# open-policy-agent/gatekeeper

Measured on AMD Instinct MI355X. Metric: AdmissionReview x constraint evals/sec, higher is better.
Workload: dtype u32; 1 GPU; configs[2]: pkg/audit sweep, 50 constraints x 1000000 mixed synthetic cluster objects (80% Pod, 10% Deployment, 5% Namespace, 5% Service/ConfigMap); constraints=50, reviews_total=1000000, reviews_rank0=1000000, rows_rank0=15859334, table_bytes_rank0=529437232, parallelism=1 GPU

## Files before the change

gatekeeper_amd/_lib.py:

```python
from __future__ import annotations

import atexit
import ctypes as C
import os

_HERE = os.path.dirname(os.path.abspath(__file__))
_ROOT = os.path.dirname(_HERE)

GK_OK = 0
GK_ERR_INVALID, GK_ERR_REGO, GK_ERR_UNSUPPORTED, GK_ERR_NOT_FOUND, GK_ERR_DEVICE, GK_ERR_REVIEW, GK_ERR_INTERNAL, GK_ERR_LIMIT = (
    -1, -2, -3, -4, -5, -6, -7, -8)
GK_REVIEW_ADMISSION_REQUEST, GK_REVIEW_OBJECT = 0, 1
GK_SRC_EMPTY, GK_SRC_ORIGINAL, GK_SRC_GENERATED, GK_SRC_ALL, GK_SRC_INVALID = 0, 1, 2, 3, 4
GK_TABLE_KEEP_DOCS = 1
GK_TABLE_RESIDENT = 2
GK_TABLE_KEEP_TEXT = 16
GK_TABLE_PRUNED = 32
GK_TABLE_PRE_MATCHED = 64
GK_TABLE_PROCESS_AUDIT = 4
GK_TABLE_PROCESS_WEBHOOK = 8
GK_REVIEW_EXCLUDED = 1
GK_EVAL_WANT_MATCH, GK_EVAL_NO_DOWNLOAD, GK_EVAL_WANT_LIST, GK_EVAL_ASYNC, GK_EVAL_COLLECT, GK_EVAL_TIME_EACH, GK_EVAL_KERNEL_ONLY = 1, 2, 4, 8, 16, 32, 64
GK_EVAL_DEVICE_ONLY = 128
GK_SWEEP_RESULT_TOTALS = 1

EXPORTS = [
    "gk_engine_create", "gk_engine_destroy", "gk_last_error", "gk_version", "gk_template_add", "gk_template_remove",
    "gk_constraint_add", "gk_constraint_remove", "gk_data_put", "gk_data_remove", "gk_excluder_replace", "gk_excluder_excluded", "gk_table_create", "gk_table_free",
    "gk_table_eval", "gk_eval_free", "gk_render", "gk_render_error", "gk_free", "gk_dump", "gk_table_topk", "gk_topk_free",
    "gk_table_totals", "gk_totals_free", "gk_table_get_stats", "gk_batcher_start", "gk_batcher_stop", "gk_query", "gk_query_ex", "gk_query_ex2",
    "gk_resident_sweep", "gk_sweep_free", "gk_resident_review", "gk_resident_review_ex",
    "gk_comm_unique_id", "gk_comm_init", "gk_comm_destroy", "gk_comm_info", "gk_table_sweep_sharded", "gk_shard_free",
    "gk_jit_quiesce", "gk_jit_cache_stats", "gk_jit_cache_dir", "gk_jit_cache_drop_memory", "gk_host_cpus", "gk_table_create_spool", "gk_spool_info_free", "gk_debug_set",
    "gk_synth_batch_create", "gk_synth_batch_reviews", "gk_synth_batch_size", "gk_synth_batch_json_bytes", "gk_synth_batch_free", "gk_synth_query_storm", "gk_synth_query_storm_ex",
]


GK_OPT_NO_REFERENTIAL, GK_OPT_GATHER_STATS, GK_OPT_TRACE = 1, 2, 4
GK_QUERY_TRACE = 1
GK_QUERY_PRE_MATCHED = 2


class gk_opts(C.Structure):
    _fields_ = [("device", C.c_int32), ("elem_cap", C.c_uint16 * 3), ("reserved", C.c_uint16), ("flags", C.c_uint32), ("reserved2", C.c_uint32),
                ("disabled_builtins", C.POINTER(C.c_char_p)), ("n_disabled_builtins", C.c_size_t)]


class gk_review_in(C.Structure):
    _fields_ = [("kind", C.c_int32), ("source", C.c_int32),
                ("json", C.c_char_p), ("json_len", C.c_size_t),
                ("namespace_json", C.c_char_p), ("namespace_len", C.c_size_t),
                ("ns_object_json", C.c_char_p), ("ns_object_len", C.c_size_t),
                ("operation", C.c_char_p)]


class gk_eval_out(C.Structure):
# ... 139 lines not shown
    lib.gk_topk_free.restype = None
    lib.gk_comm_unique_id.argtypes = [C.c_char_p]
    lib.gk_comm_init.argtypes = [vp, C.c_char_p, C.c_int, C.c_int]
    lib.gk_comm_destroy.argtypes = [vp]
    lib.gk_comm_destroy.restype = None
    lib.gk_comm_info.argtypes = [vp, C.POINTER(C.c_int32), C.POINTER(C.c_int32)]
    lib.gk_table_sweep_sharded.argtypes = [vp, vp, u32, C.POINTER(C.POINTER(gk_shard_out))]
    lib.gk_shard_free.argtypes = [C.POINTER(gk_shard_out)]
    lib.gk_shard_free.restype = None
    if hostemu:
        lib.gk_comm_init_host.argtypes = [vp, C.c_int, C.c_int, HE_ALLGATHER, HE_ALLREDUCE, vp]
    lib.gk_resident_sweep.argtypes = [vp, u32, C.POINTER(C.POINTER(gk_sweep_out))]
    lib.gk_sweep_free.argtypes = [C.POINTER(gk_sweep_out)]
    lib.gk_sweep_free.restype = None
    lib.gk_resident_review.argtypes = [vp, C.POINTER(cp), sz, C.POINTER(vp)]
    lib.gk_batcher_start.argtypes = [vp, C.POINTER(gk_batch_opts)]
    lib.gk_batcher_stop.argtypes = [vp]
    lib.gk_batcher_stop.restype = None
    lib.gk_query.argtypes = [vp, C.POINTER(gk_review_in), C.POINTER(vp), C.POINTER(gk_query_stats)]
    lib.gk_query_ex.argtypes = [vp, C.POINTER(gk_review_in), u32, C.POINTER(vp), C.POINTER(vp), C.POINTER(gk_query_stats)]
    lib.gk_query_ex2.argtypes = [vp, C.POINTER(gk_review_in), C.POINTER(u32), sz, u32, C.POINTER(vp), C.POINTER(vp), C.POINTER(gk_query_stats)]
    lib.gk_resident_review_ex.argtypes = [vp, C.POINTER(cp), sz, C.POINTER(u32), sz, u32, C.POINTER(vp)]
    lib.gk_debug_set.argtypes = [cp, C.c_int64]
    lib.gk_table_get_stats.argtypes = [vp, C.POINTER(gk_table_stats)]
    lib.gk_table_totals.argtypes = [vp, vp, C.POINTER(C.POINTER(gk_totals_out))]
    lib.gk_totals_free.argtypes = [C.POINTER(gk_totals_out)]
    lib.gk_totals_free.restype = None
    lib.gk_synth_batch_create.argtypes = [C.c_uint64, C.c_uint64, C.c_uint64, C.c_int, C.POINTER(cp), sz, C.POINTER(vp)]
    lib.gk_synth_batch_reviews.argtypes = [vp]
    lib.gk_synth_batch_reviews.restype = C.POINTER(gk_review_in)
    lib.gk_synth_batch_size.argtypes = [vp]
    lib.gk_synth_batch_size.restype = sz
    lib.gk_synth_batch_json_bytes.argtypes = [vp]
    lib.gk_synth_batch_json_bytes.restype = C.c_uint64
    lib.gk_synth_batch_free.argtypes = [vp]
    lib.gk_synth_batch_free.restype = None
    lib.gk_synth_query_storm.argtypes = [vp, vp, u32, u32, C.POINTER(gk_storm_out)]
    lib.gk_synth_query_storm_ex.argtypes = [vp, vp, u32, u32, C.POINTER(u32), sz, u32, C.POINTER(gk_storm_out)]
    atexit.register(lib.gk_jit_quiesce)
    _cache[hostemu] = lib
    return lib
```

gatekeeper_amd/csrc/device.hpp:

```cpp
#pragma once
#include <cstdint>
#include <string>
#include <vector>

#include "flatten.hpp"
#include "lower.hpp"

namespace gk {

struct DevTable;
struct DevPlan;

struct EvalOptions {
  bool download = true;
  bool want_match = false;
  uint32_t list_capacity = 0;
  bool shard = false;
  bool detached = false;
  bool kernel_only = false;
  bool time_each = false;
  bool timed = true;
  bool jit_wait = true;
};

// ... 39 lines not shown
int dev_comm_rank(const DevComm* c);
int dev_comm_world(const DevComm* c);
bool dev_comm_query(const DevComm* c, int* rank, int* world, std::string* err);
struct ShardInfo {
  uint32_t stride_tiles = 0;
  uint64_t slot_bytes = 0;
  std::vector<uint32_t> shard_reviews;
};
void dev_shard_setup(DevTable* t, DevComm* c, uint32_t nc, ShardInfo* info);
void dev_shard_exchange(DevTable* t, DevComm* c, uint32_t nc, uint64_t not_evaluated, std::vector<int64_t>* totals,
                        std::vector<uint64_t>* gathered , const void** d_gathered);
struct ShardExchangeStats { float exchange_ms = 0; uint64_t inbound_bytes = 0; bool overlap = false; };
ShardExchangeStats dev_shard_exchange_stats(const DevTable* t, const DevComm* c);
void dev_shard_enqueue(const DevPlan* p, DevTable* t, DevComm* c, const EvalOptions& opt, uint32_t nc, uint64_t not_evaluated, bool allow_graph);
bool dev_shard_collect(DevTable* t, DevComm* c, uint32_t nc, std::vector<int64_t>* totals, std::vector<uint64_t>* gathered, const void** d_gathered);
void dev_jit_quiesce();
void dev_jit_cache_stats(uint64_t* hits, uint64_t* compiles);
void dev_jit_cache_drop_memory();
const char* dev_jit_cache_dir();
void dev_jit_prefetch(const DevPlan* p, const DevTable* t);
void dev_eval_launch(const DevPlan* p, const DevTable* t, const EvalOptions& opt);
void dev_eval_finish(const DevPlan* p, const DevTable* t, const EvalOptions& opt, EvalOut* out);

}
```

gatekeeper_amd/csrc/engine.cpp:

```cpp
#include <atomic>
#include <cstring>
#include <dirent.h>
#include <algorithm>
#include <chrono>
#include <condition_variable>
#include <deque>
#include <functional>
#include <thread>
#include <map>
#include <unordered_map>
#include <unordered_set>
#include <memory>
#include <mutex>
#include <shared_mutex>
#include <sstream>

#include "../../include/gkgpu.h"
#include "codegen.hpp"
#include "device.hpp"
#include "flatten.hpp"
#include "lower.hpp"
#include "pe.hpp"
#include "regex.hpp"

// ... 232 lines not shown
    bool is_namespace = false, alive = true;
    uint32_t chunk = UINT32_MAX, slot = 0;
  };
  struct ResChunk {
    gk_table* table = nullptr;
    std::vector<uint32_t> obj_of_slot;
    std::vector<uint64_t> live;
    std::vector<uint64_t> shown;
    uint64_t excl_gen = 0;
    gk_eval_out* ev = nullptr;
    uint64_t plan_gen = 0;
    uint64_t n_live = 0;
  };
  struct Resident {
    std::mutex mu;
    std::vector<ResObj> objs;
    std::unordered_map<std::string, uint32_t> by_key;
    std::unordered_map<std::string, std::vector<uint32_t>> by_ns;
    std::unordered_map<uint64_t, uint32_t> by_text;
    std::vector<uint32_t> pending;
    std::vector<ResChunk> chunks;
    bool swept = false;
    uint64_t n_live = 0, n_dead_slots = 0, flattened_total = 0;
  } resident;
  struct BatchResult;
  struct Request {
    const gk_review_in* in = nullptr;
    bool pre_matched = false;
    std::chrono::steady_clock::time_point arrived;
    int status = GK_OK;
    std::string error;
    std::shared_ptr<BatchResult> batch;
    uint32_t index = 0;
    uint32_t batch_size = 0;
    double queue_us = 0, device_us = 0;
    bool done = false;
    std::condition_variable cv;
  };
  struct Batcher {
    std::mutex mu;
    std::condition_variable cv;
    std::deque<Request*> queue;
    std::vector<std::thread> workers;
    bool running = false, stop = false;
    gk_batch_opts opts{64, 200, 0, 0};
    uint64_t batches = 0, reviews = 0;
// ... 2006 lines not shown
        c.obj_of_slot.push_back(id);
      }
      R.pending.clear();
      if (!ins.empty()) {
        std::vector<int32_t> st(ins.size(), GK_OK);
        int rc = gk_table_create(e, ins.data(), ins.size(), GK_TABLE_RESIDENT | GK_TABLE_PRUNED, st.data(), &c.table);
        if (rc != GK_OK) return rc;
        c.live.assign((ins.size() + 63) / 64, 0);
        for (size_t k = 0; k < ins.size(); k++) {
          gk_engine::ResObj& o = R.objs[c.obj_of_slot[k]];
          o.chunk = (uint32_t)R.chunks.size(); o.slot = (uint32_t)k;
          if (st[k] == GK_OK) { c.live[k / 64] |= 1ull << (k % 64); c.n_live++; }
        }
        flattened = ins.size();
        R.flattened_total += flattened;
        R.chunks.push_back(std::move(c));
      }
    }
    const auto t1 = std::chrono::steady_clock::now();
    ensure_plan(e);
    uint64_t gen;
    { std::shared_lock<std::shared_mutex> l(e->plan_rw); gen = e->plan_gen; }
    std::unique_ptr<SweepHolder> h(new SweepHolder());
    for (auto& c : R.chunks) {
      if (c.ev && c.plan_gen == gen) continue;
      if (c.ev) { gk_eval_free(c.ev); c.ev = nullptr; }
      int rc = gk_table_eval(e, c.table, 0, &c.ev);
      if (rc != GK_OK) return rc;
      c.plan_gen = gen;
    }
    {
      std::shared_lock<std::shared_mutex> l(e->mu);
      auto ex = e->excluder.find("audit");
      for (auto& c : R.chunks) {
        if (c.excl_gen == e->excluder_gen && c.shown.size() == c.live.size()) {
          for (size_t w = 0; w < c.live.size(); w++) c.shown[w] &= c.live[w];
          continue;
        }
        c.shown = c.live;
        if (ex != e->excluder.end() && !ex->second.empty())
          for (size_t k = 0; k < c.obj_of_slot.size(); k++) {
            const gk_engine::ResObj& o = R.objs[c.obj_of_slot[k]];
            if (excluder_matches(ex->second, o.is_namespace ? o.path.back() : o.ns)) c.shown[k / 64] &= ~(1ull << (k % 64));
          }
        c.excl_gen = e->excluder_gen;
      }
    }
    if (!R.chunks.empty()) {
      const gk_eval_out* ev0 = R.chunks[0].ev;
      h->ids.assign(ev0->constraint_ids, ev0->constraint_ids + ev0->n_constraints);
    } else {
      { std::lock_guard<std::mutex> gate(e->plan_gate); }
// ... 293 lines not shown
    stats->total_us = std::chrono::duration<double, std::micro>(std::chrono::steady_clock::now() - req.arrived).count();
  }
  if (req.status != GK_OK) return fail(req.status, req.error);
  char* buf = (char*)malloc(results.size() + 1);
  memcpy(buf, results.c_str(), results.size() + 1);
  *results_json = buf;
  gk_query_stats mine{};
  mine.batch_size = req.batch_size; mine.queue_us = req.queue_us; mine.device_us = req.device_us;
  put_trace(on_host ? (pre_matched ? "by the host evaluator (the review is beyond the device's limits; pre-matched by the caller: violation sets by the concrete evaluator)"
                                   : "by the host evaluator (the review is beyond the device's limits: match layer from the stripped review on the device, violation sets by the concrete evaluator)")
                    : (pre_matched ? "on the device (pre-matched by the caller: violation bitmaps of the batch's one launch; messages rendered by the host evaluator for the flagged pairs)"
                                   : "on the device (match + violation bitmaps of the batch's one launch; messages rendered by the host evaluator for the flagged pairs)"), results, &mine);
  return GK_OK;
}

int gk_debug_set(const char* key, int64_t value) {
  if (!key) return fail(GK_ERR_INVALID, "NULL argument");
  if (strcmp(key, "dict_facts") == 0) { g_debug_dict_facts.store(value != 0); return GK_OK; }
  if (strcmp(key, "group_max") == 0) { g_debug_group_max.store((int)std::max<int64_t>(0, std::min<int64_t>(value, 1 << 20))); return GK_OK; }
  if (strcmp(key, "fold_match_labels") == 0) { g_test_fold_match_labels.store(value != 0); return GK_OK; }
  return fail(GK_ERR_NOT_FOUND, std::string("gk_debug_set: unknown key ") + key);
}

void gk_jit_quiesce(void) { dev_jit_quiesce(); }
void gk_jit_cache_drop_memory(void) { dev_jit_cache_drop_memory(); }
const char* gk_jit_cache_dir(void) { return dev_jit_cache_dir(); }
void gk_jit_cache_stats(uint64_t* cache_hits, uint64_t* compiles) {
  uint64_t h = 0, c = 0;
  dev_jit_cache_stats(&h, &c);
  if (cache_hits) *cache_hits = h;
  if (compiles) *compiles = c;
}

int gk_dump(gk_engine* e, char** text_out) {
  if (!e || !text_out) return fail(GK_ERR_INVALID, "NULL argument");
  try {
    ensure_plan(e);
    std::ostringstream os;
    std::shared_lock<std::shared_mutex> l(e->plan_rw);
    const HostPlan& p = e->fast;
    os << "constraints=" << p.dims.n_constraints << " viol_formulas=" << p.n_viol << " match_formulas=" << p.n_match
       << " preds=" << p.dims.n_preds << " scopes=" << p.dims.n_scopes << " code_words=" << p.dims.n_code
       << " gwords=" << p.dims.n_gwords << " acc_words=" << p.dims.acc_words << " lds_bytes_per_64_reviews=" << p.dims.acc_words * 256
       << " paths=" << p.dims.n_paths << "\n";
    for (size_t i = 0; i < p.preds.size(); i++)
      os << "pred " << i << " op=" << (int)p.preds[i].op << " dst=" << (int)p.preds[i].dst << " scope=" << (int)p.preds[i].scope
// ... 15 lines not shown
```

gatekeeper_amd/csrc/kernels.hip:

```cpp
#include <hip/hip_runtime.h>
#include <hip/hiprtc.h>
#include <dlfcn.h>
#include <sys/stat.h>
#include <sys/wait.h>
#include <spawn.h>
#include <unistd.h>
#include <fcntl.h>
#include <array>
#include <cstring>
#include <cerrno>
#include <set>

#include <cstdio>
#include <cstdlib>
#include <atomic>
#include <condition_variable>
#include <list>
#include <map>
#include <thread>
#include <memory>
#include <mutex>
#include <stdexcept>
#include <string>
#include <vector>

extern char** environ;

#include "chunks.hpp"
#include "codegen.hpp"
#include "device.hpp"
#include "jit_source.hpp"
#include "shard_pipe.hpp"
#include "jit_sources.inc"
#include "vm_core.hpp"

namespace gk {

#define HIP_OK(expr)                                                                                          \
  do {                                                                                                        \
    hipError_t e_ = (expr);                                                                                   \
    if (e_ != hipSuccess) throw std::runtime_error(std::string("HIP error: ") + hipGetErrorString(e_) + " at " #expr); \
  } while (0)

namespace {
struct DevPool {
  std::mutex mu;
  std::map<size_t, std::vector<void*>> free_;
  std::map<void*, size_t> class_of;
  size_t cached = 0;
};
DevPool& pool() { static DevPool p; return p; }
constexpr size_t kPoolMaxBlock = 32u << 20, kPoolMaxCached = 2048ull << 20;
std::mutex g_hip_alloc_mu;
hipError_t hip_malloc_serial(void** out, size_t bytes) { std::lock_guard<std::mutex> l(g_hip_alloc_mu); return hipMalloc(out, bytes); }
void hip_free_serial(void* p) { std::lock_guard<std::mutex> l(g_hip_alloc_mu); (void)hipFree(p); }
// ... 899 lines not shown
  void lc_release_more() {
    for (size_t k = 0; k < lc_more.size(); k++) { if (lc_pinned) pinned_release(reinterpret_cast<uint8_t*>(lc_more[k]), lc_more_cap[k]); else pool_free(lc_more[k]); }
    lc_more.clear(); lc_more_cap.clear(); lc_used = 0;
  }
  struct Launch {
    uint64_t plan = 0;
    bool want_match = false;
    hipFunction_t fn = nullptr;
    uint32_t grid = 0, block = 0, lds = 0, tot_k = 0;
    uint64_t kernel_hash = 0;
    PlanView pv{};
    const Row* rows = nullptr; const StrHdr* shdr = nullptr; const ChunkDesc* lists = nullptr; const uint32_t* rflags = nullptr; const uint8_t* heap = nullptr;
    const ConstraintSlot* slots = nullptr;
    uint32_t cg = 0, nn = 0, nt = 0, dd = 0, rp = 0;
    OutPtrs out{};
  } cached;
  bool timed = false;
  size_t timed_from = 0;
  void open_bracket(size_t launch_no, bool want, hipStream_t stream) {
    if (launch_no == 0) timed = false;
    if (want && !timed) { HIP_OK(hipEventRecord(ev_first, stream)); timed = true; timed_from = launch_no; }
  }
  hipEvent_t ev_first = nullptr, ev_last = nullptr;
  std::vector<std::pair<hipEvent_t, hipEvent_t>> evs;
  size_t pending = 0;
  bool lc_dirty = false;
  bool per_launch = false;
  uint32_t lds_bytes = 0;
  hipEvent_t ev_x0 = nullptr, ev_x1 = nullptr;
  float exchange_ms = 0;
  uint64_t kernel_hash = 0;
  uint8_t* h_pin = nullptr;
  size_t pin_cap = 0;
  uint8_t* pinned(size_t bytes) {
    if (bytes > pin_cap) {
      pinned_release(h_pin, pin_cap);
      h_pin = pinned_acquire(bytes, &pin_cap);
    }
    return h_pin;
  }
  void release() {
    drop_graph();
    cached.plan = 0;
    lc_release_more();
    pool_free(own_viol ? d_viol : nullptr); pool_free(d_err); pool_free(d_match); pool_free(d_ovf); pool_free(d_big); pool_free(d_list); if (lc_pinned) pinned_release(reinterpret_cast<uint8_t*>(d_lc), lc_pin_cap); else pool_free(d_lc); lc_pinned = false; pool_free(d_done); pool_free(d_partial);
    d_viol = d_err = d_match = d_ovf = d_big = nullptr; d_counts = d_list = d_lc = d_done = d_partial = nullptr; partial_cap = partial_rows = 0; partial_live = false; last_lc = nullptr;
  }
  ~Work() { drop_graph(); release(); pinned_release(h_pin, pin_cap); shard_teardown(); pool_free(d_totals); for (auto& e : evs) { hipEventDestroy(e.first); hipEventDestroy(e.second); } if (ev_first) hipEventDestroy(ev_first); if (ev_last) hipEventDestroy(ev_last); if (ev_x0) hipEventDestroy(ev_x0); if (ev_x1) hipEventDestroy(ev_x1); }
};

static bool host_atomics_work(int device) {
  static std::mutex mu;
  static std::map<int, bool> known;
  std::lock_guard<std::mutex> l(mu);
  auto it = known.find(device);
  if (it == known.end()) {
    int v = 0;
    if (hipDeviceGetAttribute(&v, hipDeviceAttributeHostNativeAtomicSupported, device) != hipSuccess) { (void)hipGetLastError(); v = 0; }
    it = known.emplace(device, v != 0).first;
  }
  return it->second;
}

static Work* get_work(const DevTable* t, uint32_t nc, uint32_t n_tiles, const EvalOptions& opt) {
  DevTable* mt = const_cast<DevTable*>(t);
  if (!mt->work) mt->work = new Work();
  Work* w = mt->work;
  bool want_match = opt.want_match;
  if (opt.shard && (!w->d_all || w->shard_nc != nc || w->stride_tiles != n_tiles)) throw std::runtime_error("sharded evaluation without dev_shard_setup for this plan");
  if (w->nc != nc || w->n_tiles != n_tiles || w->list_cap < opt.list_capacity || (want_match && !w->has_match) || w->own_viol == opt.shard) {
    if (w->d_err) (void)hipStreamSynchronize(t->stream);
    w->release();
// ... 90 lines not shown
  uint32_t rpp = rpt;
  const size_t dyn_cap = p->want_jit ? max_dyn_lds_jit(rpt, p->res_k, 0, jit_tot_k(p->n_constraints)) : max_dyn_lds_of(rpt);
  while (rpp > (uint32_t)GK_TILE && (size_t)p->fast.dims.acc_words * rpp * 4 > dyn_cap) rpp /= 2;
  if (const char* f = getenv("GK_FORCE_RPP")) rpp = std::min<uint32_t>(rpt, std::max<uint32_t>(GK_TILE, (uint32_t)atoi(f)));
  uint32_t jit_lcap = list_cap_of(jit_block_of(rpt));
  if (p->want_jit && rpt >= 256) {
    DevTable* mt = const_cast<DevTable*>(t);
    if (mt->chunk_need_plan != p->id) { mt->chunk_need = chunk_need(p, t); mt->chunk_need_plan = p->id; }
    jit_lcap = jit_list_cap(jit_block_of(rpt), mt->chunk_need);
  }
  *rpp_out = rpp; *lcap_out = jit_lcap;
}

void dev_jit_prefetch(const DevPlan* p, const DevTable* t) {
  if (!p || !t || !p->want_jit || t->n_reviews == 0 || p->n_constraints == 0) return;
  uint32_t rpp = 0, lcap = 0;
  jit_geometry(p, t, &rpp, &lcap);
  try { (void)jit_for(const_cast<DevPlan*>(p), t->rpt, rpp, t, false, lcap, true); } catch (const std::exception&) {}
}

static uint32_t* lc_for_launch(Work* w, const EvalOptions& opt, hipStream_t stream) {
  if (opt.detached) return w->d_lc + Work::LC_WORDS * Work::LC_SLOTS;
  if (w->lc_dirty && w->pending == 0) {
    w->lc_zero_used([&](uint32_t* at, size_t bytes) { HIP_OK(hipMemsetAsync(at, 0, bytes, stream)); });
    w->lc_dirty = false;
  }
  const size_t i = w->pending;
  while (i / Work::LC_SLOTS > w->lc_more.size()) {
    uint32_t* blk = nullptr;
    size_t cap = 0;
    if (w->lc_pinned) {
      blk = reinterpret_cast<uint32_t*>(pinned_acquire(Work::LC_SLOTS * Work::LC_BYTES, &cap));
      if (!blk) throw std::runtime_error("no pinned memory for the launch counters");
      memset(blk, 0, Work::LC_SLOTS * Work::LC_BYTES);
    } else {
      HIP_OK(pool_malloc(&blk, Work::LC_SLOTS * Work::LC_BYTES));
      HIP_OK(hipMemsetAsync(blk, 0, Work::LC_SLOTS * Work::LC_BYTES, stream));
    }
    w->lc_more.push_back(blk); w->lc_more_cap.push_back(cap);
  }
  return w->lc_slot(i);
}

void dev_eval_launch(const DevPlan* p, const DevTable* t, const EvalOptions& opt) {
  const uint32_t n = t->n_reviews, nc = p->n_constraints;
  const uint32_t n_tiles = opt.shard && t->work ? t->work->stride_tiles : (n + GK_TILE - 1) / GK_TILE;
  if (n == 0 || nc == 0) return;
  if (Work* cw = t->work; cw && cw->cached.plan == p->id && cw->cached.want_match == opt.want_match && !opt.shard && !opt.detached && !opt.time_each &&
                          opt.list_capacity == 0) {
    Work::Launch& c = cw->cached;
    hipStream_t stream = t->stream;
    c.out.list_count = cw->last_lc = lc_for_launch(cw, opt, stream);
    cw->open_bracket(cw->pending++, opt.timed, stream);
    cw->per_launch = false;
    cw->partial_rows = c.grid; cw->partial_stride = c.tot_k; cw->partial_live = true;
    cw->lds_bytes = c.lds; cw->kernel_hash = c.kernel_hash;
    void* args[] = {&c.pv, &c.rows, &c.shdr, &c.lists, &c.cg, &c.rflags, &c.heap, &c.nn, &c.nt, &c.slots, &c.out, &c.dd, &c.rp};
    HIP_OK(hipModuleLaunchKernel(c.fn, c.grid, 1, 1, c.block, 1, 1, c.lds, stream, args, nullptr));
    return;
  }
  Work* w = get_work(t, nc, n_tiles, opt);
  w->cached.plan = 0;
  hipStream_t stream = t->stream;
  if (opt.shard && !opt.detached && w->overlap && w->comm_stream) { HIP_OK(hipStreamSynchronize(w->comm_stream)); w->pipe.pending[0] = w->pipe.pending[1] = false; }
  uint32_t* lc = lc_for_launch(w, opt, stream);
  w->last_lc = lc;
  static const bool want_prof = getenv("GK_KERNEL_PROF") != nullptr;
  if (want_prof && !w->d_prof) { HIP_OK(pool_malloc(&w->d_prof, ((size_t)n / GK_RPT_MIN + 8) * 64)); HIP_OK(hipMemsetAsync(w->d_prof, 0, ((size_t)n / GK_RPT_MIN + 8) * 64, stream)); }
  OutPtrs out{w->d_viol, w->d_err, opt.want_match ? w->d_match : nullptr, w->d_ovf, w->d_big, w->d_counts, w->d_list, lc,
              opt.list_capacity, w->d_prof, nullptr};
  const bool per_launch = !opt.detached && opt.time_each;
  if (!w->ev_first) { HIP_OK(hipEventCreate(&w->ev_first)); HIP_OK(hipEventCreate(&w->ev_last)); }
  if (per_launch && w->pending == w->evs.size()) {
    hipEvent_t a, b;
    HIP_OK(hipEventCreate(&a)); HIP_OK(hipEventCreate(&b));
    w->evs.emplace_back(a, b);
  }
  const size_t launch_no = opt.detached ? ~(size_t)0 : w->pending++;
  const uint32_t rpt = t->rpt;
  int block = gk_block_of((int)rpt);
  const uint32_t n_groups = (n + rpt - 1) / rpt;
  static const uint32_t dbg_phase = getenv("GK_DBG_PHASE") ? (uint32_t)atoi(getenv("GK_DBG_PHASE")) : 0u;
  static const uint32_t stagger = getenv("GK_STAGGER") ? (uint32_t)atoi(getenv("GK_STAGGER")) & 0xFFFu : (uint32_t)GK_STAGGER_DEFAULT;
  constexpr uint32_t stagger_mode = 0u;
  uint32_t rpp = rpt, jit_lcap = 0;
// ... 29 lines not shown
  if (jit && jit->tot_k) {
    if ((size_t)w->partial_cap < (size_t)grid_full * jit->tot_k) {
      if (w->d_partial) { w->drop_graph(); HIP_OK(hipStreamSynchronize(stream)); pool_free(w->d_partial); w->d_partial = nullptr; }
      w->partial_cap = ((grid_full + 255u) / 256u * 256u) * jit->tot_k;
      HIP_OK(pool_malloc(&w->d_partial, (size_t)w->partial_cap * 4));
    }
    out.partial = w->d_partial;
    if (!opt.detached) { w->partial_rows = grid; w->partial_stride = jit->tot_k; }
  }
  if (!opt.detached) w->partial_live = fused_totals;
  w->lds_bytes = (uint32_t)lds;
  w->kernel_hash = jit ? jit->source_hash : 0;
  if (per_launch) { HIP_OK(hipEventRecord(w->evs[launch_no].first, stream)); if (launch_no == 0) w->timed = false; }
  else if (!opt.detached) w->open_bracket(launch_no, opt.timed, stream);
  if (!opt.detached) w->per_launch = per_launch;
  if (jit) {
    PlanView pv = p->fast.view();
    const Row* rows = t->rows; const StrHdr* shdr = t->shdr; const uint32_t* rflags = t->rflags;
    const uint8_t* heap = t->heap;
    const ChunkDesc* lists = t->bind_fast.lists;
    uint32_t nn = n, nt = n_tiles, dd = dbg, cg = t->bind_fast.capg, rp = rpp;
    const ConstraintSlot* slots = p->slots;
    void* args[] = {&pv, &rows, &shdr, &lists, &cg, &rflags, &heap, &nn, &nt, &slots, &out, &dd, &rp};
    HIP_OK(hipModuleLaunchKernel(jit->tiles, grid, 1, 1, block, 1, 1, (unsigned)lds, stream, args, nullptr));
    if (fused_totals && !opt.detached && !per_launch && opt.list_capacity == 0 && !w->d_prof) {
      Work::Launch& c = w->cached;
      c.want_match = opt.want_match; c.fn = jit->tiles; c.grid = grid; c.block = (uint32_t)block; c.lds = (uint32_t)lds;
      c.tot_k = jit->tot_k; c.kernel_hash = jit->source_hash; c.pv = pv; c.rows = rows; c.shdr = shdr; c.lists = lists; c.rflags = rflags; c.heap = heap;
      c.slots = slots; c.cg = cg; c.nn = nn; c.nt = nt; c.dd = dd; c.rp = rp; c.out = out;
      c.plan = p->id;
    }
  } else {
    auto fn = rpt == 64 ? gk_eval_tiles_64 : rpt == 128 ? gk_eval_tiles_128 : rpt == 256 ? gk_eval_tiles_256 : gk_eval_tiles_512;
    hipLaunchKernelGGL(fn, dim3(grid), dim3(block), lds, stream, p->fast.view(), t->rows, t->shdr, t->bind_fast.lists, t->bind_fast.capg,
                       t->rflags, t->heap, n, n_tiles, p->slots, out, dbg, rpp);
    HIP_OK(hipGetLastError());
  }
  if (per_launch) HIP_OK(hipEventRecord(w->evs[launch_no].second, stream));
  if (!opt.shard && !opt.kernel_only && !fused_totals) launch_count_rows(w->d_viol, nc, n_tiles, w->d_counts, stream, 0, true);
}

void dev_eval_finish(const DevPlan* p, const DevTable* t, const EvalOptions& opt, EvalOut* o) {
  const uint32_t n = t->n_reviews, nc = p->n_constraints;
  const uint32_t n_tiles = opt.shard && t->work ? t->work->stride_tiles : (n + GK_TILE - 1) / GK_TILE;
  o->n_reviews = n; o->n_constraints = nc; o->n_tiles = n_tiles;
  o->kernel_ms = o->fast_kernel_ms = 0;
  o->n_overflow = 0; o->list_total = 0; o->n_launches = 0;
  if (n == 0 || nc == 0) {
    o->viol.assign((size_t)nc * n_tiles, 0); o->err = o->viol; o->match = o->viol; o->too_big.assign(n_tiles, 0); o->counts.assign(nc, 0); o->list.clear();
    return;
  }
  Work* w = t->work;
  if (!w || w->pending == 0) throw std::runtime_error("dev_eval_finish without a pending launch");
  hipStream_t stream = t->stream;
  const size_t bm_words = (size_t)nc * n_tiles;
  uint32_t lc[2] = {0, 0};
  if (!w->per_launch && w->timed) HIP_OK(hipEventRecord(w->ev_last, stream));
  uint32_t* d_lc_last = w->lc_slot(w->pending - 1);
  if (w->partial_live && !opt.shard) launch_sum_partials(w->d_partial, w->partial_rows, w->partial_stride, nc, w->d_counts, stream);
  if (w->lc_pinned) {
    HIP_OK(hipStreamSynchronize(stream));
    memcpy(lc, d_lc_last, 8);
  } else if (uint8_t* pin0 = w->pinned(64)) {
    HIP_OK(hipMemcpyAsync(pin0, d_lc_last, 8, hipMemcpyDeviceToHost, stream));
    HIP_OK(hipStreamSynchronize(stream));
    memcpy(lc, pin0, 8);
  } else {
    HIP_OK(hipMemcpyAsync(lc, d_lc_last, 8, hipMemcpyDeviceToHost, stream));
    HIP_OK(hipStreamSynchronize(stream));
  }
  float total = 0;
  if (w->per_launch) { for (size_t i = 0; i < w->pending; i++) { float ms = 0; HIP_OK(hipEventElapsedTime(&ms, w->evs[i].first, w->evs[i].second)); total += ms; } }
  else if (w->timed) HIP_OK(hipEventElapsedTime(&total, w->ev_first, w->ev_last));
  o->n_launches = (uint32_t)w->pending;
  w->lc_used = std::max(w->lc_used, w->pending);
  o->lds_bytes = w->lds_bytes;
  o->kernel_hash = w->kernel_hash;
// ... 160 lines not shown
                                                      uint32_t* __restrict__ lc, uint32_t zero_lc) {
  __shared__ uint32_t partial[16];
  const uint32_t r = blockIdx.x;
  const uint64_t* row = r < nc ? viol + (size_t)r * stride : r < 2u * nc ? err + (size_t)(r - nc) * stride : big;
  const uint32_t sum = gk_row_popcount(row, n_words, partial);
  if (threadIdx.x != 0) return;
  unsigned long long* t64 = reinterpret_cast<unsigned long long*>(tail + (size_t)nc * 8);
  if (r < 2u * nc) reinterpret_cast<uint32_t*>(tail)[r] = sum;
  else t64[0] = sum;
  if (r == 0) {
    t64[1] = not_evaluated;
    t64[2] = lc ? (unsigned long long)lc[1] : 0ull;
    if (lc && zero_lc) { lc[0] = 0; lc[1] = 0; }
  }
}

static size_t shard_tail_off(uint32_t nc, uint32_t stride) { return (size_t)nc * stride * 8; }
static size_t shard_slot_bytes(uint32_t nc, uint32_t stride) { return (shard_tail_off(nc, stride) + (size_t)nc * 8 + 8 * GK_TAIL_EXTRA + 15) & ~(size_t)15; }

void dev_shard_setup(DevTable* t, DevComm* c, uint32_t nc, ShardInfo* info) {
  HIP_OK(hipSetDevice(c->device));
  if (!t->work) t->work = new Work();
  Work* w = t->work;
  unsigned long long* d_sizes;
  HIP_OK(pool_malloc(&d_sizes, (size_t)c->world * 8));
  const unsigned long long mine = t->n_reviews;
  HIP_OK(hipMemcpy(d_sizes + c->rank, &mine, 8, hipMemcpyHostToDevice));
  NCCL_OK(c, c->lib->AllGather(d_sizes + c->rank, d_sizes, 8, kNcclUint8, c->comm, t->stream));
  HIP_OK(hipStreamSynchronize(t->stream));
  std::vector<unsigned long long> sizes(c->world);
  HIP_OK(hipMemcpy(sizes.data(), d_sizes, (size_t)c->world * 8, hipMemcpyDeviceToHost));
  pool_free(d_sizes);
  info->shard_reviews.clear();
  uint32_t stride = 1;
  for (int r = 0; r < c->world; r++) { info->shard_reviews.push_back((uint32_t)sizes[r]); stride = std::max<uint32_t>(stride, (uint32_t)((sizes[r] + GK_TILE - 1) / GK_TILE)); }
  info->stride_tiles = stride;
  info->slot_bytes = shard_slot_bytes(nc, stride);
  w->drop_graph();
  w->shard_teardown();
  pool_free(w->d_totals);
  w->d_totals = nullptr;
  w->release();
  w->nc = 0;
  w->overlap = false;
  if (const char* ov = getenv("GK_SHARD_OVERLAP")) w->overlap = atoi(ov) != 0;
  w->shard_device = c->device;
// ... 94 lines not shown
  hipStream_t stream = t->stream;
  HIP_OK(hipStreamSynchronize(stream));
  if (w->overlap && w->comm_stream) { HIP_OK(hipStreamSynchronize(w->comm_stream)); w->pipe.pending[0] = w->pipe.pending[1] = false; }
  totals->resize(2 * (size_t)nc + GK_TAIL_EXTRA);
  HIP_OK(hipMemcpy(totals->data(), w->d_totals, (2 * (size_t)nc + GK_TAIL_EXTRA) * 8, hipMemcpyDeviceToHost));
  if (gathered) {
    gathered->resize((size_t)c->world * w->slot_bytes / 8);
    HIP_OK(hipMemcpy(gathered->data(), w->d_all, (size_t)c->world * w->slot_bytes, hipMemcpyDeviceToHost));
  }
  if (d_gathered) *d_gathered = w->d_all;
}

bool dev_shard_collect(DevTable* t, DevComm* c, uint32_t nc, std::vector<int64_t>* totals, std::vector<uint64_t>* gathered, const void** d_gathered) {
  Work* w = t->work;
  if (!w || !w->d_all || w->shard_nc != nc || w->shard_not_eval == ~0ull) return false;
  std::vector<int64_t> tot;
  shard_download(t, c, nc, &tot, nullptr, nullptr);
  if (tot[2 * (size_t)nc + 2] != 0) return false;
  shard_download(t, c, nc, totals, gathered, d_gathered);
  return true;
}

void dev_shard_enqueue(const DevPlan* p, DevTable* t, DevComm* c, const EvalOptions& opt, uint32_t nc, uint64_t not_evaluated, bool allow_graph) {
  static const bool graph_on = getenv("GK_SHARD_GRAPH") && atoi(getenv("GK_SHARD_GRAPH")) != 0;
  Work* w = t->work;
  const bool use_graph = graph_on && allow_graph && !(w && w->overlap);
  const uint64_t key = (p->id << 20) ^ ((uint64_t)nc << 8) ^ not_evaluated ^ ((uint64_t)t->n_reviews << 32);
  hipStream_t stream = t->stream;
  if (use_graph && w && w->graph_state == 2 && w->graph_key == key) { HIP_OK(hipGraphLaunch(w->graph_exec, stream)); w->last_lc = w->d_lc + Work::LC_WORDS * Work::LC_SLOTS; return; }
  if (use_graph && w && w->graph_state == 1 && w->graph_key == key && t->n_reviews != 0 && nc != 0) {
    hipGraph_t graph = nullptr;
    bool ok = hipStreamBeginCapture(stream, hipStreamCaptureModeRelaxed) == hipSuccess;
    if (ok) {
      try {
        EvalOptions co = opt;
        co.detached = true;
        dev_eval_launch(p, t, co);
        shard_exchange_enqueue(t, c, nc, not_evaluated);
      } catch (const std::exception&) { ok = false; }
      if (hipStreamEndCapture(stream, &graph) != hipSuccess || !graph) ok = false;
    }
    if (ok && hipGraphInstantiate(&w->graph_exec, graph, nullptr, nullptr, 0) != hipSuccess) { ok = false; w->graph_exec = nullptr; }
    if (graph) hipGraphDestroy(graph);
    (void)hipGetLastError();
    if (ok) { w->graph_state = 2; HIP_OK(hipGraphLaunch(w->graph_exec, stream)); w->last_lc = w->d_lc + Work::LC_WORDS * Work::LC_SLOTS; return; }
    w->graph_state = -1;
// ... 1 lines not shown
    if (!told) { told = true; fprintf(stderr, "[gkgpu] sharded sweep: graph capture failed, enqueuing directly\n"); }
  }
  EvalOptions eo = opt;
  eo.detached = true;
  if (w && w->overlap) {
    Work::HipShardBackend be{p, t, c, eo, nc, not_evaluated};
    w->pipe.enqueue(be);
    return;
  }
  dev_eval_launch(p, t, eo);
  shard_exchange_enqueue(t, c, nc, not_evaluated);
  w = t->work;
  if (use_graph && w && (w->graph_state == 0 || (w->graph_state > 0 && w->graph_key != key))) {
    if (w->graph_exec) { hipGraphExecDestroy(w->graph_exec); w->graph_exec = nullptr; }
    w->graph_state = 1; w->graph_key = key;
  }
}

void dev_topk(const DevTable* t, uint32_t nc, const std::vector<uint32_t>& order, const std::vector<uint32_t>& grp, uint32_t k, uint32_t cap,
              std::vector<uint32_t>* idx, std::vector<uint32_t>* n, std::vector<uint32_t>* ovf) {
  idx->assign((size_t)nc * cap, 0xFFFFFFFFu); n->assign(nc, 0); ovf->assign(nc, 0);
  Work* w = t->work;
  if (!w || !w->d_viol || w->nc != nc) throw std::runtime_error("dev_topk: evaluate the table first");
  if (nc == 0 || t->n_reviews == 0 || k == 0) return;
  uint32_t* d_order = upload(order.data(), order.size());
  uint32_t* d_grp = upload(grp.data(), grp.size());
  uint32_t *d_idx = nullptr, *d_n = nullptr, *d_ovf = nullptr;
  HIP_OK(pool_malloc(&d_idx, (size_t)nc * cap * 4));
  HIP_OK(hipMemsetAsync(d_idx, 0xFF, (size_t)nc * cap * 4, t->stream));
  HIP_OK(pool_malloc(&d_n, (size_t)nc * 4));
  HIP_OK(pool_malloc(&d_ovf, (size_t)nc * 4));
  hipLaunchKernelGGL(gk_topk_rows, dim3(nc), dim3(GK_TILE), 0, t->stream, w->d_viol, w->n_tiles, d_order, d_grp, t->n_reviews, k, cap, d_idx, d_n, d_ovf);
  HIP_OK(hipGetLastError());
  HIP_OK(hipStreamSynchronize(t->stream));
  HIP_OK(hipMemcpy(idx->data(), d_idx, (size_t)nc * cap * 4, hipMemcpyDeviceToHost));
  HIP_OK(hipMemcpy(n->data(), d_n, (size_t)nc * 4, hipMemcpyDeviceToHost));
  HIP_OK(hipMemcpy(ovf->data(), d_ovf, (size_t)nc * 4, hipMemcpyDeviceToHost));
  pool_free(d_order); pool_free(d_grp); pool_free(d_idx); pool_free(d_n); pool_free(d_ovf);
}

void dev_last_viol(const DevTable* t, uint32_t nc, std::vector<uint64_t>* viol) {
  viol->clear();
  Work* w = t->work;
  if (!w || !w->d_viol || w->nc != nc) return;
  viol->resize((size_t)nc * w->n_tiles);
  HIP_OK(hipStreamSynchronize(t->stream));
  if (!viol->empty()) HIP_OK(hipMemcpy(viol->data(), w->d_viol, viol->size() * 8, hipMemcpyDeviceToHost));
}

void dev_eval(const DevPlan* p, const DevTable* t, const EvalOptions& opt, EvalOut* o) {
  dev_eval_launch(p, t, opt);
  dev_eval_finish(p, t, opt, o);
}

}
```

include/gkgpu.h:

```cpp
#ifndef GKGPU_H
#define GKGPU_H
#include <stddef.h>
#include <stdint.h>

#ifdef __cplusplus
extern "C" {
#endif

typedef struct gk_engine gk_engine;
typedef struct gk_table gk_table;

typedef enum {
  GK_OK = 0,
  GK_ERR_INVALID = -1,
  GK_ERR_REGO = -2,
  GK_ERR_UNSUPPORTED = -3,
  GK_ERR_NOT_FOUND = -4,
  GK_ERR_DEVICE = -5,
  GK_ERR_REVIEW = -6,
  GK_ERR_INTERNAL = -7,
  GK_ERR_LIMIT = -8
} gk_status;

#define GK_OPT_NO_REFERENTIAL 1u
// ... 190 lines not shown
typedef struct {
  uint32_t batch_size;
  uint32_t reserved;
  double queue_us;
  double device_us;
  double total_us;
} gk_query_stats;
int gk_batcher_start(gk_engine* e, const gk_batch_opts* opts);
void gk_batcher_stop(gk_engine* e);
int gk_query(gk_engine* e, const gk_review_in* review, char** results_json, gk_query_stats* stats);
#define GK_QUERY_TRACE 1u
int gk_query_ex(gk_engine* e, const gk_review_in* review, uint32_t flags, char** results_json, char** trace_out, gk_query_stats* stats);
#define GK_QUERY_PRE_MATCHED 2u
int gk_query_ex2(gk_engine* e, const gk_review_in* review, const uint32_t* constraint_ids, size_t n_constraints, uint32_t flags,
                 char** results_json, char** trace_out, gk_query_stats* stats);

void gk_jit_quiesce(void);
void gk_jit_cache_stats(uint64_t* cache_hits, uint64_t* compiles);
const char* gk_jit_cache_dir(void);
void gk_jit_cache_drop_memory(void);

int gk_debug_set(const char* key, int64_t value);

int gk_dump(gk_engine* e, char** text_out);

#ifdef __cplusplus
}
#endif
#endif
```

Baseline: 1382 billion evals/s.

## Enqueue resident sweep chunks asynchronously and add optional second launch stream

The resident sweep now launches every stale chunk asynchronously before collecting results, instead of evaluating each chunk synchronously in turn. This lets device work for later chunks queue behind earlier ones and hides per-chunk host round trips. Separately, an env-gated mode deals repeated cached launches alternately onto a second HIP stream, with fork/join events inserted before any dependent operation. This adds synchronization complexity and debug counters, and the second-stream path is off by default.

Measured after the change: 1384 billion evals/s (median of 2 runs). Within noise of the previous version (+0.2%).

```diff
diff --git a/gatekeeper_amd/_lib.py b/gatekeeper_amd/_lib.py
--- a/gatekeeper_amd/_lib.py
+++ b/gatekeeper_amd/_lib.py
@@ -31,7 +31,7 @@
     "gk_table_totals", "gk_totals_free", "gk_table_get_stats", "gk_batcher_start", "gk_batcher_stop", "gk_query", "gk_query_ex", "gk_query_ex2",
     "gk_resident_sweep", "gk_sweep_free", "gk_resident_review", "gk_resident_review_ex",
     "gk_comm_unique_id", "gk_comm_init", "gk_comm_destroy", "gk_comm_info", "gk_table_sweep_sharded", "gk_shard_free",
-    "gk_jit_quiesce", "gk_jit_cache_stats", "gk_jit_cache_dir", "gk_jit_cache_drop_memory", "gk_host_cpus", "gk_table_create_spool", "gk_spool_info_free", "gk_debug_set",
+    "gk_jit_quiesce", "gk_jit_cache_stats", "gk_jit_cache_dir", "gk_jit_cache_drop_memory", "gk_host_cpus", "gk_table_create_spool", "gk_spool_info_free", "gk_debug_set", "gk_debug_sweep_streams", "gk_debug_resident_sweep",
     "gk_synth_batch_create", "gk_synth_batch_reviews", "gk_synth_batch_size", "gk_synth_batch_json_bytes", "gk_synth_batch_free", "gk_synth_query_storm", "gk_synth_query_storm_ex",
 ]
 
@@ -217,6 +217,8 @@
     lib.gk_query_ex2.argtypes = [vp, C.POINTER(gk_review_in), C.POINTER(u32), sz, u32, C.POINTER(vp), C.POINTER(vp), C.POINTER(gk_query_stats)]
     lib.gk_resident_review_ex.argtypes = [vp, C.POINTER(cp), sz, C.POINTER(u32), sz, u32, C.POINTER(vp)]
     lib.gk_debug_set.argtypes = [cp, C.c_int64]
+    lib.gk_debug_sweep_streams.argtypes = [vp, u32, C.POINTER(C.c_uint64)]
+    lib.gk_debug_resident_sweep.argtypes = [vp, C.POINTER(C.c_uint64)]
     lib.gk_table_get_stats.argtypes = [vp, C.POINTER(gk_table_stats)]
     lib.gk_table_totals.argtypes = [vp, vp, C.POINTER(C.POINTER(gk_totals_out))]
     lib.gk_totals_free.argtypes = [C.POINTER(gk_totals_out)]
diff --git a/gatekeeper_amd/csrc/device.hpp b/gatekeeper_amd/csrc/device.hpp
--- a/gatekeeper_amd/csrc/device.hpp
+++ b/gatekeeper_amd/csrc/device.hpp
@@ -85,4 +85,6 @@
 void dev_eval_launch(const DevPlan* p, const DevTable* t, const EvalOptions& opt);
 void dev_eval_finish(const DevPlan* p, const DevTable* t, const EvalOptions& opt, EvalOut* out);
 
+void dev_sweep_stats(const DevTable* t, uint64_t out[3]);
+
 }
diff --git a/gatekeeper_amd/csrc/engine.cpp b/gatekeeper_amd/csrc/engine.cpp
--- a/gatekeeper_amd/csrc/engine.cpp
+++ b/gatekeeper_amd/csrc/engine.cpp
@@ -278,6 +278,7 @@
     std::vector<ResChunk> chunks;
     bool swept = false;
     uint64_t n_live = 0, n_dead_slots = 0, flattened_total = 0;
+    uint64_t last_enqueued = 0, last_enqueued_first = 0;
   } resident;
   struct BatchResult;
   struct Request {
@@ -2330,12 +2331,22 @@
     uint64_t gen;
     { std::shared_lock<std::shared_mutex> l(e->plan_rw); gen = e->plan_gen; }
     std::unique_ptr<SweepHolder> h(new SweepHolder());
+    R.last_enqueued = R.last_enqueued_first = 0;
+    std::vector<gk_engine::ResChunk*> stale;
     for (auto& c : R.chunks) {
       if (c.ev && c.plan_gen == gen) continue;
       if (c.ev) { gk_eval_free(c.ev); c.ev = nullptr; }
-      int rc = gk_table_eval(e, c.table, 0, &c.ev);
+      gk_eval_out* none = nullptr;
+      int rc = gk_table_eval(e, c.table, GK_EVAL_ASYNC, &none);
       if (rc != GK_OK) return rc;
-      c.plan_gen = gen;
+      stale.push_back(&c);
+      R.last_enqueued++;
+    }
+    for (gk_engine::ResChunk* c : stale) {
+      if (c == stale.front()) R.last_enqueued_first = R.last_enqueued;
+      int rc = gk_table_eval(e, c->table, GK_EVAL_COLLECT, &c->ev);
+      if (rc != GK_OK) return rc;
+      c->plan_gen = gen;
     }
     {
       std::shared_lock<std::shared_mutex> l(e->mu);
@@ -2675,6 +2686,20 @@
   return fail(GK_ERR_NOT_FOUND, std::string("gk_debug_set: unknown key ") + key);
 }
 
+int gk_debug_sweep_streams(const gk_table* t, uint32_t workspace, uint64_t out[3]) {
+  if (!t || !out) return fail(GK_ERR_INVALID, "NULL argument");
+  if (workspace > t->views.size()) return fail(GK_ERR_NOT_FOUND, "gk_debug_sweep_streams: no such workspace");
+  dev_sweep_stats(workspace == 0 ? t->dev : t->views[workspace - 1], out);
+  return GK_OK;
+}
+
+int gk_debug_resident_sweep(gk_engine* e, uint64_t out[2]) {
+  if (!e || !out) return fail(GK_ERR_INVALID, "NULL argument");
+  std::lock_guard<std::mutex> rl(e->resident.mu);
+  out[0] = e->resident.last_enqueued; out[1] = e->resident.last_enqueued_first;
+  return GK_OK;
+}
+
 void gk_jit_quiesce(void) { dev_jit_quiesce(); }
 void gk_jit_cache_drop_memory(void) { dev_jit_cache_drop_memory(); }
 const char* gk_jit_cache_dir(void) { return dev_jit_cache_dir(); }
diff --git a/gatekeeper_amd/csrc/kernels.hip b/gatekeeper_amd/csrc/kernels.hip
--- a/gatekeeper_amd/csrc/kernels.hip
+++ b/gatekeeper_amd/csrc/kernels.hip
@@ -31,6 +31,7 @@
 #include "device.hpp"
 #include "jit_source.hpp"
 #include "shard_pipe.hpp"
+#include "sweep_streams.hpp"
 #include "jit_sources.inc"
 #include "vm_core.hpp"
 
@@ -976,6 +977,27 @@
     if (want && !timed) { HIP_OK(hipEventRecord(ev_first, stream)); timed = true; timed_from = launch_no; }
   }
   hipEvent_t ev_first = nullptr, ev_last = nullptr;
+  SweepDeal deal;
+  hipStream_t stream2 = nullptr;
+  int stream2_device = 0;
+  hipEvent_t ev_join = nullptr, ev_fork = nullptr;
+  bool fork_pending = false;
+  void fork(hipStream_t table_stream) {
+    if (!sweep_two_streams() || !table_stream) return;
+    if (!ev_fork) HIP_OK(hipEventCreateWithFlags(&ev_fork, hipEventDisableTiming));
+    HIP_OK(hipEventRecord(ev_fork, table_stream));
+    fork_pending = true;
+  }
+  hipStream_t second(int device) {
+    if (!stream2) {
+      stream2 = stream_acquire(device);
+      if (!stream2) throw std::runtime_error("no second launch stream for the sweeps");
+      stream2_device = device;
+    }
+    if (!ev_join) HIP_OK(hipEventCreateWithFlags(&ev_join, hipEventDisableTiming));
+    if (fork_pending) { HIP_OK(hipStreamWaitEvent(stream2, ev_fork, 0)); fork_pending = false; }
+    return stream2;
+  }
   std::vector<std::pair<hipEvent_t, hipEvent_t>> evs;
   size_t pending = 0;
   bool lc_dirty = false;
@@ -1000,8 +1022,24 @@
     pool_free(own_viol ? d_viol : nullptr); pool_free(d_err); pool_free(d_match); pool_free(d_ovf); pool_free(d_big); pool_free(d_list); if (lc_pinned) pinned_release(reinterpret_cast<uint8_t*>(d_lc), lc_pin_cap); else pool_free(d_lc); lc_pinned = false; pool_free(d_done); pool_free(d_partial);
     d_viol = d_err = d_match = d_ovf = d_big = nullptr; d_counts = d_list = d_lc = d_done = d_partial = nullptr; partial_cap = partial_rows = 0; partial_live = false; last_lc = nullptr;
   }
-  ~Work() { drop_graph(); release(); pinned_release(h_pin, pin_cap); shard_teardown(); pool_free(d_totals); for (auto& e : evs) { hipEventDestroy(e.first); hipEventDestroy(e.second); } if (ev_first) hipEventDestroy(ev_first); if (ev_last) hipEventDestroy(ev_last); if (ev_x0) hipEventDestroy(ev_x0); if (ev_x1) hipEventDestroy(ev_x1); }
+  ~Work() {
+    if (stream2) { stream_release(stream2_device, stream2); stream2 = nullptr; }
+    if (ev_join) hipEventDestroy(ev_join);
+    if (ev_fork) hipEventDestroy(ev_fork);
+    drop_graph(); release(); pinned_release(h_pin, pin_cap); shard_teardown(); pool_free(d_totals); for (auto& e : evs) { hipEventDestroy(e.first); hipEventDestroy(e.second); } if (ev_first) hipEventDestroy(ev_first); if (ev_last) hipEventDestroy(ev_last); if (ev_x0) hipEventDestroy(ev_x0); if (ev_x1) hipEventDestroy(ev_x1);
+  }
 };
+
+static void sweep_join(const DevTable* t) {
+  Work* w = t ? t->work : nullptr;
+  if (!w || !w->deal.join()) return;
+  HIP_OK(hipEventRecord(w->ev_join, w->stream2));
+  HIP_OK(hipStreamWaitEvent(t->stream, w->ev_join, 0));
+}
+void dev_sweep_stats(const DevTable* t, uint64_t out[3]) {
+  out[0] = out[1] = out[2] = 0;
+  if (t && t->work) { out[0] = t->work->deal.n_first; out[1] = t->work->deal.n_second; out[2] = t->work->deal.n_joins; }
+}
 
 static bool host_atomics_work(int device) {
   static std::mutex mu;
@@ -1138,8 +1176,10 @@
 static uint32_t* lc_for_launch(Work* w, const EvalOptions& opt, hipStream_t stream) {
   if (opt.detached) return w->d_lc + Work::LC_WORDS * Work::LC_SLOTS;
   if (w->lc_dirty && w->pending == 0) {
+    const bool any = w->lc_used != 0;
     w->lc_zero_used([&](uint32_t* at, size_t bytes) { HIP_OK(hipMemsetAsync(at, 0, bytes, stream)); });
     w->lc_dirty = false;
+    if (any) w->fork(stream);
   }
   const size_t i = w->pending;
   while (i / Work::LC_SLOTS > w->lc_more.size()) {
@@ -1152,6 +1192,7 @@
     } else {
       HIP_OK(pool_malloc(&blk, Work::LC_SLOTS * Work::LC_BYTES));
       HIP_OK(hipMemsetAsync(blk, 0, Work::LC_SLOTS * Work::LC_BYTES, stream));
+      w->fork(stream);
     }
     w->lc_more.push_back(blk); w->lc_more_cap.push_back(cap);
   }
@@ -1162,12 +1203,23 @@
   const uint32_t n = t->n_reviews, nc = p->n_constraints;
   const uint32_t n_tiles = opt.shard && t->work ? t->work->stride_tiles : (n + GK_TILE - 1) / GK_TILE;
   if (n == 0 || nc == 0) return;
-  if (Work* cw = t->work; cw && cw->cached.plan == p->id && cw->cached.want_match == opt.want_match && !opt.shard && !opt.detached && !opt.time_each &&
-                          opt.list_capacity == 0) {
+  Work* cw = t->work;
+  const SweepWay way = cw ? sweep_way(cw->cached.plan, cw->cached.want_match, cw->pending, cw->timed, t->stream != nullptr, p->id, opt) : SweepWay{false, false};
+  if (way.short_way) {
     Work::Launch& c = cw->cached;
+    if (!way.indep) sweep_join(t);
+    const int lane = way.indep ? cw->deal.next() : 0;
     hipStream_t stream = t->stream;
-    c.out.list_count = cw->last_lc = lc_for_launch(cw, opt, stream);
-    cw->open_bracket(cw->pending++, opt.timed, stream);
+    if (lane) {
+      if (!(c.plan == p->id && c.want_match == opt.want_match && c.tot_k >= nc && c.out.partial && !c.out.list_capacity && !c.out.prof && !cw->d_prof &&
+            !(cw->pending && cw->timed) && !opt.shard && !opt.detached && !opt.time_each && !opt.timed))
+        throw std::logic_error("a pass that is not independent was dealt to the second launch stream");
+      stream = cw->second(t->device);
+    }
+    c.out.list_count = cw->last_lc = lc_for_launch(cw, opt, t->stream);
+    if (lane && cw->fork_pending) stream = cw->second(t->device);
+    cw->open_bracket(cw->pending++, opt.timed, t->stream);
+    cw->deal.took(lane);
     cw->per_launch = false;
     cw->partial_rows = c.grid; cw->partial_stride = c.tot_k; cw->partial_live = true;
     cw->lds_bytes = c.lds; cw->kernel_hash = c.kernel_hash;
@@ -1175,8 +1227,10 @@
     HIP_OK(hipModuleLaunchKernel(c.fn, c.grid, 1, 1, c.block, 1, 1, c.lds, stream, args, nullptr));
     return;
   }
+  sweep_join(t);
   Work* w = get_work(t, nc, n_tiles, opt);
   w->cached.plan = 0;
+  w->deal.first();
   hipStream_t stream = t->stream;
   if (opt.shard && !opt.detached && w->overlap && w->comm_stream) { HIP_OK(hipStreamSynchronize(w->comm_stream)); w->pipe.pending[0] = w->pipe.pending[1] = false; }
   uint32_t* lc = lc_for_launch(w, opt, stream);
@@ -1252,8 +1306,10 @@
     uint32_t nn = n, nt = n_tiles, dd = dbg, cg = t->bind_fast.capg, rp = rpp;
     const ConstraintSlot* slots = p->slots;
     void* args[] = {&pv, &rows, &shdr, &lists, &cg, &rflags, &heap, &nn, &nt, &slots, &out, &dd, &rp};
+    const bool repeatable = sweep_repeatable(fused_totals, per_launch, w->d_prof != nullptr, opt);
+    if (repeatable) w->fork(stream);
     HIP_OK(hipModuleLaunchKernel(jit->tiles, grid, 1, 1, block, 1, 1, (unsigned)lds, stream, args, nullptr));
-    if (fused_totals && !opt.detached && !per_launch && opt.list_capacity == 0 && !w->d_prof) {
+    if (repeatable) {
       Work::Launch& c = w->cached;
       c.want_match = opt.want_match; c.fn = jit->tiles; c.grid = grid; c.block = (uint32_t)block; c.lds = (uint32_t)lds;
       c.tot_k = jit->tot_k; c.kernel_hash = jit->source_hash; c.pv = pv; c.rows = rows; c.shdr = shdr; c.lists = lists; c.rflags = rflags; c.heap = heap;
@@ -1283,6 +1339,7 @@
   Work* w = t->work;
   if (!w || w->pending == 0) throw std::runtime_error("dev_eval_finish without a pending launch");
   hipStream_t stream = t->stream;
+  sweep_join(t);
   const size_t bm_words = (size_t)nc * n_tiles;
   uint32_t lc[2] = {0, 0};
   if (!w->per_launch && w->timed) HIP_OK(hipEventRecord(w->ev_last, stream));
@@ -1489,6 +1546,7 @@
   HIP_OK(hipSetDevice(c->device));
   if (!t->work) t->work = new Work();
   Work* w = t->work;
+  sweep_join(t);
   unsigned long long* d_sizes;
   HIP_OK(pool_malloc(&d_sizes, (size_t)c->world * 8));
   const unsigned long long mine = t->n_reviews;
@@ -1629,6 +1687,7 @@
 }
 
 void dev_shard_enqueue(const DevPlan* p, DevTable* t, DevComm* c, const EvalOptions& opt, uint32_t nc, uint64_t not_evaluated, bool allow_graph) {
+  sweep_join(t);
   static const bool graph_on = getenv("GK_SHARD_GRAPH") && atoi(getenv("GK_SHARD_GRAPH")) != 0;
   Work* w = t->work;
   const bool use_graph = graph_on && allow_graph && !(w && w->overlap);
@@ -1676,6 +1735,7 @@
   idx->assign((size_t)nc * cap, 0xFFFFFFFFu); n->assign(nc, 0); ovf->assign(nc, 0);
   Work* w = t->work;
   if (!w || !w->d_viol || w->nc != nc) throw std::runtime_error("dev_topk: evaluate the table first");
+  sweep_join(t);
   if (nc == 0 || t->n_reviews == 0 || k == 0) return;
   uint32_t* d_order = upload(order.data(), order.size());
   uint32_t* d_grp = upload(grp.data(), grp.size());
@@ -1698,6 +1758,7 @@
   Work* w = t->work;
   if (!w || !w->d_viol || w->nc != nc) return;
   viol->resize((size_t)nc * w->n_tiles);
+  sweep_join(t);
   HIP_OK(hipStreamSynchronize(t->stream));
   if (!viol->empty()) HIP_OK(hipMemcpy(viol->data(), w->d_viol, viol->size() * 8, hipMemcpyDeviceToHost));
 }
diff --git a/gatekeeper_amd/csrc/sweep_streams.hpp b/gatekeeper_amd/csrc/sweep_streams.hpp
--- /dev/null
+++ b/gatekeeper_amd/csrc/sweep_streams.hpp
@@ -0,0 +1,45 @@
+#pragma once
+#include <cstdint>
+#include <cstdlib>
+
+#include "device.hpp"
+
+namespace gk {
+
+inline bool sweep_two_streams() {
+  static const bool on = getenv("GK_SWEEP_STREAMS") && atoi(getenv("GK_SWEEP_STREAMS")) == 2;
+  return on;
+}
+
+inline bool sweep_plain(const EvalOptions& o) { return !o.shard && !o.detached && !o.time_each && !o.timed && o.list_capacity == 0; }
+
+struct SweepWay { bool short_way, indep; };
+inline SweepWay sweep_way(uint64_t cached_plan, bool cached_match, size_t pending, bool bracket_open, bool has_stream, uint64_t plan, const EvalOptions& o) {
+  const bool short_way = cached_plan != 0 && cached_plan == plan && cached_match == o.want_match && !o.shard && !o.detached && !o.time_each && o.list_capacity == 0;
+  return SweepWay{short_way, short_way && sweep_plain(o) && !(pending && bracket_open) && has_stream};
+}
+inline bool sweep_repeatable(bool fused_totals, bool per_launch, bool phase_marks, const EvalOptions& o) {
+  return fused_totals && !o.detached && !per_launch && o.list_capacity == 0 && !phase_marks;
+}
+inline bool sweep_opens_bracket(bool per_launch, const EvalOptions& o) { return !o.detached && !per_launch && o.timed; }
+
+struct SweepDeal {
+  uint32_t run = 0;
+  uint32_t on_second = 0;
+  uint64_t n_first = 0, n_second = 0, n_joins = 0;
+  int next() const { return sweep_two_streams() ? (int)(run & 1u) : 0; }
+  void took(int s) {
+    run++;
+    if (s) { on_second++; n_second++; } else n_first++;
+  }
+  void first() { took(0); }
+  bool join() {
+    run = 0;
+    if (!on_second) return false;
+    on_second = 0;
+    n_joins++;
+    return true;
+  }
+};
+
+}
diff --git a/include/gkgpu.h b/include/gkgpu.h
--- a/include/gkgpu.h
+++ b/include/gkgpu.h
@@ -236,6 +236,9 @@
 
 int gk_debug_set(const char* key, int64_t value);
 
+int gk_debug_sweep_streams(const gk_table* table, uint32_t workspace, uint64_t out[3]);
+int gk_debug_resident_sweep(gk_engine* e, uint64_t out[2]);
+
 int gk_dump(gk_engine* e, char** text_out);
 
 #ifdef __cplusplus
```
